# NightShade99/Self-Supervised-Vision

Hardware: AMD Instinct MI355X
Metric: images/sec (whole node) SimCLR ResNet-50 two-view train step (higher is better)
Workload: dtype f32; 1 GPU; SimCLR resnet50 (7x7/2 stem) synthetic 3x224x224, bs=512/GPU, global batch 512, NT-Xent(normalize, T=0.5) over the global batch, SGD-Nesterov; per_gpu_batch=512, global_batch=512, params=27971008, parallelism=single, view_streams=2, library=self-supervised-vision_amd/csrc/libssv_hip.so

## Files before the change

### include/ssv_hip.h

```cpp
#ifndef SSV_HIP_H
#define SSV_HIP_H

#include <stddef.h>
#include <stdint.h>

#ifdef __cplusplus
extern "C" {
#endif

typedef enum ssv_status {
  SSV_OK = 0,
  SSV_ERR_INVALID = -1,
  SSV_ERR_WORKSPACE = -2,
  SSV_ERR_LAUNCH = -3
} ssv_status;

int ssv_version(void);
const char* ssv_last_error(void);
const char* ssv_source_sha16(void);
int ssv_device_cus(void);

typedef struct ssv_conv_desc {
  int32_t N, H, W, C;
  int32_t K, R, S;
  int32_t stride, pad;
  int32_t Ho, Wo;
  int32_t arithmetic;
  int32_t reserved;
  const void* w_planes;
} ssv_conv_desc;
enum { SSV_ARITH_F32_MFMA = 0, SSV_ARITH_BF16X3 = 6 };
int ssv_conv_arithmetic(const ssv_conv_desc* d, int32_t product);
int ssv_split_planes(int64_t n, const float* x, void* planes, void* stream);

int ssv_conv2d_fwd(const ssv_conv_desc* d, const float* x, const float* w, const float* bias,
                   const float* addend, float* y, void* stream);
int ssv_pad_channels(int64_t npix, int32_t cin, int32_t cout, const float* in, float* out, int32_t accumulate, void* stream);
int ssv_group_expand(int32_t K, int32_t R, int32_t S, int32_t Cg, int32_t groups, const float* wg, float* wd, void* stream);
int ssv_group_extract(int32_t K, int32_t R, int32_t S, int32_t Cg, int32_t groups, const float* dwd, float* dwg, int32_t accumulate, void* stream);

int ssv_conv2d_fwd_grouped(const ssv_conv_desc* d, int32_t groups, const float* x, const float* wd, const float* bias, const float* addend,
                           float* y, void* stream);
int ssv_conv2d_dgrad_grouped(const ssv_conv_desc* d, int32_t groups, const float* dy, const float* wd, const float* addend, float* dx, void* stream);
size_t ssv_conv2d_wgrad_grouped_workspace_bytes(const ssv_conv_desc* d, int32_t groups);
int ssv_conv2d_wgrad_grouped(const ssv_conv_desc* d, int32_t groups, const float* x, const float* dy, float* dwd, int accumulate,
                             void* ws, size_t ws_bytes, void* stream);
int ssv_filter_transpose(int32_t K, int32_t R, int32_t S, int32_t C, const float* w, float* wt, void* stream);
int64_t ssv_conv2d_fwd_stats_groups(const ssv_conv_desc* d);
int ssv_conv2d_fwd_stats(const ssv_conv_desc* d, const float* x, const float* w, float* y, float* pmean, float* pm2, void* stream);
int ssv_conv2d_fwd_bnrelu_in_stats(const ssv_conv_desc* d, const float* x, const float* in_scale, const float* in_shift,
                                   const float* w, float* y, float* pmean, float* pm2, void* stream);
int ssv_conv2d_wgrad_bnrelu_in(const ssv_conv_desc* d, const float* x, const float* in_scale, const float* in_shift, const float* dy,
                               float* dw, int accumulate, void* ws, size_t ws_bytes, void* stream);
typedef struct ssv_bn_gate {
  const float* x;
  const float* scale;
  const float* shift;
  const uint8_t* mask;
  const float* mean;
  const float* invstd;
  float* psum_g;
  float* psum_gx;
  const float* x2;
  const float* mean2;
  const float* invstd2;
// ... 274 lines not shown
```

### self-supervised-vision_amd/_lib.py

```python
import ctypes as C
import os

import torch

_HERE = os.path.dirname(os.path.abspath(__file__))
LIB_PATH = os.environ.get("SSV_HIP_LIB") or os.path.join(_HERE, "csrc", "libssv_hip.so")

ABI_VERSION = 121
PROF_CLASSES = ("conv_fwd", "conv_dgrad", "conv_wgrad", "bn_fwd", "bn_bwd", "pool", "loss", "optim", "aug", "misc", "attn", "norm")


class SsvError(RuntimeError):
    pass


ARITH_F32_MFMA, ARITH_BF16X3 = 0, 6


class ConvDesc(C.Structure):
    _fields_ = [(n, C.c_int32) for n in ("N", "H", "W", "C", "K", "R", "S", "stride", "pad", "Ho", "Wo", "arithmetic", "reserved")] + [("w_planes", C.c_void_p)]


class BnGate(C.Structure):
    _fields_ = [(n, C.c_void_p) for n in ("x", "scale", "shift", "mask", "mean", "invstd", "psum_g", "psum_gx", "x2", "mean2", "invstd2", "psum_gx2")]


class BnDyin(C.Structure):
    _fields_ = [(n, C.c_void_p) for n in ("x", "coef")]


class AugCfg(C.Structure):
    _fields_ = [(n, C.c_double) for n in ("brightness", "contrast", "saturation", "hue", "p_jitter", "p_gray", "p_flip",
                                          "scale_min", "scale_max", "ratio_min", "ratio_max")]


_vp, _i32, _i64, _f32, _sz = C.c_void_p, C.c_int32, C.c_int64, C.c_float, C.c_size_t
_u64 = C.c_uint64
_f3 = C.POINTER(C.c_float)
_cd = C.POINTER(ConvDesc)

SIGNATURES = {
    "ssv_version": (C.c_int, []),
    "ssv_last_error": (C.c_char_p, []),
    "ssv_source_sha16": (C.c_char_p, []),
    "ssv_device_cus": (C.c_int, []),
    "ssv_conv2d_fwd": (C.c_int, [_cd, _vp, _vp, _vp, _vp, _vp, _vp]),
    "ssv_pad_channels": (C.c_int, [_i64, _i32, _i32, _vp, _vp, _i32, _vp]),
    "ssv_group_expand": (C.c_int, [_i32, _i32, _i32, _i32, _i32, _vp, _vp, _vp]),
    "ssv_group_extract": (C.c_int, [_i32, _i32, _i32, _i32, _i32, _vp, _vp, _i32, _vp]),
    "ssv_conv2d_fwd_stats_groups": (_i64, [_cd]),
    "ssv_conv2d_fwd_stats": (C.c_int, [_cd, _vp, _vp, _vp, _vp, _vp, _vp]),
    "ssv_conv2d_fwd_bnrelu_in_stats": (C.c_int, [_cd, _vp, _vp, _vp, _vp, _vp, _vp, _vp, _vp]),
    "ssv_conv2d_fwd_sumin_stats": (C.c_int, [_cd] + [_vp] * 13),
    "ssv_conv2d_wgrad_bnrelu_in": (C.c_int, [_cd, _vp, _vp, _vp, _vp, _vp, C.c_int, _vp, _sz, _vp]),
    "ssv_bn_stats_finalize": (C.c_int, [_i64, _i32, _vp, _vp, _i32, _vp, _vp, _f32, _f32, _vp, _vp, _vp, _vp, _vp, _vp, _vp, _vp, _sz, _vp]),
    "ssv_bn_apply": (C.c_int, [_i64, _i32, _vp, _vp, _vp, _vp, _vp, _vp, C.c_int, _vp, _vp, _vp]),
    "ssv_bn_relu_bwd_affine": (C.c_int, [_i64, _i32, _vp, _vp, _vp, _vp, _vp, _vp, _vp, _vp, _vp, _vp, C.c_int, _vp, _sz, _vp]),
    "ssv_bn_train_fwd_partials": (C.c_int, [_i64, _i32, _vp, _vp, _vp, _i32, _vp, _vp, _vp, C.c_int, _f32, _f32, _vp, _vp, _vp, _vp, _vp, _vp, _vp, _vp, _sz, _vp]),
    "ssv_filter_transpose": (C.c_int, [_i32, _i32, _i32, _i32, _vp, _vp, _vp]),
    "ssv_conv2d_dgrad": (C.c_int, [_cd, _vp, _vp, _vp, _vp, _vp]),
    "ssv_conv2d_fwd_gate_groups": (_i64, [_cd]),
    "ssv_conv2d_fwd_gated": (C.c_int, [_cd, _vp, _vp, _vp, _vp, C.POINTER(BnGate), _vp]),
    "ssv_conv2d_fwd_gated_s2add": (C.c_int, [_cd, _vp, _vp, _vp, _i32, _i32, _vp, C.POINTER(BnGate), _vp]),
    "ssv_conv2d_fwd_dyin_s2add": (C.c_int, [_cd, _vp, C.POINTER(BnDyin), _vp, _vp, _i32, _i32, _vp, C.POINTER(BnGate), _vp]),
    "ssv_conv2d_dgrad_gate_groups": (_i64, [_cd]),
    "ssv_conv2d_dgrad_gated": (C.c_int, [_cd, _vp, _vp, _vp, _vp, C.POINTER(BnGate), _vp]),
    "ssv_bn_bwd_from_partials": (C.c_int, [_i64, _i32, _vp, _vp, _vp, _vp, _vp, _vp, _vp, _i64, _vp, _vp, _vp, C.c_int, _vp, _sz, _vp]),
    "ssv_bn_bwd_coef": (C.c_int, [_i64, _i32, _vp, _vp, _vp, _vp, _vp, _i64, _vp, _vp, _vp, C.c_int, _vp, _sz, _vp]),
    "ssv_conv2d_fwd_dyin": (C.c_int, [_cd, _vp, C.POINTER(BnDyin), _vp, _vp, _vp, C.POINTER(BnGate), _vp]),
    "ssv_conv2d_wgrad_dyin": (C.c_int, [_cd, _vp, _vp, _vp, _vp, C.POINTER(BnDyin), _vp, C.c_int, _vp, _sz, _vp]),
    "ssv_conv2d_wgrad_workspace_bytes": (_sz, [_cd]),
    "ssv_conv2d_fwd_grouped": (C.c_int, [_cd, _i32, _vp, _vp, _vp, _vp, _vp, _vp]),
    "ssv_conv2d_dgrad_grouped": (C.c_int, [_cd, _i32, _vp, _vp, _vp, _vp, _vp]),
    "ssv_conv2d_wgrad_grouped_workspace_bytes": (_sz, [_cd, _i32]),
    "ssv_conv2d_wgrad_grouped": (C.c_int, [_cd, _i32, _vp, _vp, _vp, C.c_int, _vp, _sz, _vp]),
    "ssv_conv2d_wgrad": (C.c_int, [_cd, _vp, _vp, _vp, C.c_int, _vp, _sz, _vp]),
    "ssv_conv2d_wgrad_bias_workspace_bytes": (_sz, [_cd]),
    "ssv_conv2d_wgrad_bias": (C.c_int, [_cd, _vp, _vp, _vp, _vp, C.c_int, _vp, _sz, _vp]),
    "ssv_stem_conv_fwd": (C.c_int, [_cd, _vp, _vp, _vp, _vp, _vp, _vp]),
    "ssv_stem_conv_fwd_stats_rows_per_group": (_i64, [_cd]),
    "ssv_stem_conv_wgrad_rows_per_group": (_i64, [_cd]),
    "ssv_stem_conv_wgrad_workspace_bytes": (_sz, [_cd]),
    "ssv_stem_conv_wgrad": (C.c_int, [_cd, _vp, _vp, _vp, _vp, _sz, _vp]),
# ... 204 lines not shown
```

### self-supervised-vision_amd/csrc/conv_mfma.hip

```cpp
#include "common.h"
#include "split_bf16.h"
#include <string.h>
#include <type_traits>

namespace {

constexpr int GBK = 16;

__device__ __forceinline__ int xcd_remap(int orig, int nwg) {
  const int q = nwg >> 3, r = nwg & 7, xcd = orig & 7;
  return (xcd < r ? xcd * (q + 1) : r * (q + 1) + (xcd - r) * q) + (orig >> 3);
}

struct ConvKP {
  int N, H, W, C, K, R, S, stride, pad, Ho, Wo;
  int M;
  int RSC;
  FastDiv dHoWo, dWo, dC, dS, dWp;
  float* aux_out;
  float* aux_out2;
  const float* aux_in;
  const float* xf_scale;
  const float* xf_shift;
  ssv_bn_gate gate;
  const float* dyin_x;
  const float* dyin_coef;
  const float* sum_res; const float* sum_scale; const float* sum_shift; const float* sum_rscale; const float* sum_rshift;
  float* sum_out; uint8_t* sum_mask;
  long long bs_a, bs_b, bs_o;
  int add_H2, add_W2;
  int Cg, Kg;
  const unsigned short* w_planes;
  long long wp_stride;
};

__device__ __forceinline__ void group_span(int n0, int n1, int og, int ig, int bk, int ctot, int& lo, int& hi) {
  const int glo = n0 / og, ghi = (n1 - 1) / og;
  lo = glo * ig / bk * bk;
  hi = min(ctot, ((ghi + 1) * ig + bk - 1) / bk * bk);
}

constexpr int XF_MAXC = 1024;

__device__ __forceinline__ float gelu_f(float v) { return ssv_gelu(v); }
__device__ __forceinline__ float gelu_grad_f(float v) { return ssv_gelu_grad(v); }

using rsrc_t = __amdgpu_buffer_rsrc_t;
constexpr int OOB_OFF = (int)0x80000000u;
__device__ __forceinline__ rsrc_t make_rsrc(const void* base, unsigned bytes) {
  return __builtin_amdgcn_make_buffer_rsrc((void*)base, 0, bytes, 0x00020000);
}
// ... 846 lines not shown
        }
      } else {
        epilogue_vec<TM, TN, EPI>(sel_acc<(SP != 0)>(acc, acc16), smem + wave * (32 * (TN * 32 + 4)), lane, n0 + wc0, p.K, bias, addend, y, (long long)p.M * p.K,
                                  [&](int r) -> long long { const int m = rbase + r; return m < p.M ? (long long)m * p.K : -1; },
                                  (EPI == 1 || EPI == 4) ? p.aux_out : nullptr, (EPI == 2 || EPI == 5) ? p.aux_in : nullptr);
      }
      return;
    }
  }
  static_assert(GATE == 0 || (VEC && EP_FLOATS <= SMEM), "the gated epilogue is the vectorised one");
  if constexpr (SP) return;
  const int l31 = lane & 31, h = lane >> 5;
#pragma unroll
  for (int tn = 0; tn < TN; ++tn) {
    const int col = n0 + wc0 + tn * 32 + l31;
    if (col >= p.K) continue;
    const float bv = bias ? bias[col] : 0.f;
#pragma unroll
    for (int tm = 0; tm < TM; ++tm) {
#pragma unroll
      for (int j = 0; j < 16; ++j) {
        const int row = m0 + wr0 + tm * 32 + (j & 3) + 8 * (j >> 2) + 4 * h;
        if (row < p.M) {
          const size_t o = (size_t)row * p.K + col;
          float v = acc[tm][tn][j] + bv;
          if (addend) v += addend[o];
          y[o] = v;
        }
      }
    }
  }
}

template <int BM, int BN, int WGM, int WGN, int BK, bool EPI = false, int GATE = 0, bool SP = false>
__global__ void __launch_bounds__(256, SP ? 2 : 3)
conv_dgrad_k(ConvKP p, const float* __restrict__ dy, const float* __restrict__ w, const float* addend, float* dx) {
  constexpr int TM = BM / WGM / 32, TN = BN / WGN / 32;
  constexpr int LDT = BK + 4;
  static_assert(!SP || (BK == 32 && BN == 128), "the bf16-piece data gradient: K-step 32, 128 input channels per tile");
  constexpr int A_FLOATS = BM * LDT, B_FLOATS = BK * BN, STAGE = SP ? 48 * (BM + BN) : A_FLOATS + B_FLOATS;
  __shared__ __attribute__((aligned(16))) float smem[STAGE];
  __shared__ unsigned rowpix[BM];
  __shared__ int taps[64 * 3];
  __shared__ int ntaps_s;
  float* As = smem;
  float* Bs = smem + A_FLOATS;
  const int tid = threadIdx.x, lane = tid & 63, wave = tid >> 6;
  const int wr0 = (wave / WGN) * (BM / WGM), wc0 = (wave % WGN) * (BN / WGN);
  const int st = p.stride;
  const int ph = blockIdx.y / st, pw = blockIdx.y - ph * st;
  const int Hq = ph < p.H ? (p.H - ph + st - 1) / st : 0;
  const int Wq = pw < p.W ? (p.W - pw + st - 1) / st : 0;
  const int Mc = p.N * Hq * Wq;
  const int NT = (p.C + BN - 1) / BN;
  const int bid = xcd_remap(blockIdx.x, gridDim.x);
  const int mt = bid / NT, nt = bid - mt * NT;
  const int m0 = mt * BM, n0 = nt * BN;
  if (m0 >= Mc) {
    if constexpr (GATE != 0) {
      const long long grp = ((long long)blockIdx.y * (gridDim.x / NT) + mt) * (BM / 64) + (wr0 / 64);
      const int col = n0 + wc0 + lane;
      for (int c = col; c < min(n0 + wc0 + BN / WGN, p.C); c += 64) { p.gate.psum_g[grp * p.C + c] = 0.f; p.gate.psum_gx[grp * p.C + c] = 0.f; }
    }
    return;
  }

// ... 453 lines not shown
      const float c = partial[(size_t)(k + 2) * n + i], d = partial[(size_t)(k + 3) * n + i];
      s += (a + b) + (c + d);
    }
    for (; k < k1; ++k) s += partial[(size_t)k * n + i];
  }
  sm[grp][e] = s;
  __syncthreads();
  if (grp == 0 && i < n) dw[i] = (accumulate ? dw[i] : 0.f) + ((sm[0][e] + sm[1][e]) + (sm[2][e] + sm[3][e]));
}

int check_desc(const ssv_conv_desc* d, const char* who) {
  SSV_REQUIRE(d != nullptr, "%s: null descriptor", who);
  SSV_REQUIRE(d->N > 0 && d->H > 0 && d->W > 0 && d->C > 0 && d->K > 0 && d->R > 0 && d->S > 0 && d->stride > 0 && d->pad >= 0,
              "%s: non-positive dimension", who);
  const int Ho = (d->H + 2 * d->pad - d->R) / d->stride + 1, Wo = (d->W + 2 * d->pad - d->S) / d->stride + 1;
  SSV_REQUIRE(Ho == d->Ho && Wo == d->Wo, "%s: Ho/Wo (%d,%d) inconsistent with input/filter/stride/pad (expect %d,%d)", who, d->Ho, d->Wo, Ho, Wo);
  SSV_REQUIRE((int64_t)d->N * d->H * d->W < (1ll << 31) && (int64_t)d->N * d->Ho * d->Wo < (1ll << 31), "%s: too many pixels", who);
  SSV_REQUIRE((int64_t)d->R * d->S * d->C < (1 << 24) && d->R * d->S <= 64 && d->H < 32768 && d->W < 32768, "%s: filter too large", who);
  SSV_REQUIRE((int64_t)d->N * d->H * d->W * d->C < (1ll << 29) - (1 << 22) && (int64_t)d->N * d->Ho * d->Wo * d->K < (1ll << 29) - (1 << 22) &&
              (int64_t)d->K * d->R * d->S * d->C < (1ll << 29), "%s: tensor of 2 GiB or more - split the batch", who);
  return SSV_OK;
}

ConvKP make_kp(const ssv_conv_desc* d) {
  ConvKP p;
  p.N = d->N; p.H = d->H; p.W = d->W; p.C = d->C; p.K = d->K; p.R = d->R; p.S = d->S;
  p.stride = d->stride; p.pad = d->pad; p.Ho = d->Ho; p.Wo = d->Wo;
  p.M = d->N * d->Ho * d->Wo;
  p.RSC = d->R * d->S * d->C;
  p.dHoWo = make_fastdiv((uint32_t)(d->Ho * d->Wo));
  p.dWo = make_fastdiv((uint32_t)d->Wo);
  p.dC = make_fastdiv((uint32_t)d->C);
  p.dS = make_fastdiv((uint32_t)d->S);
  p.dWp = make_fastdiv((uint32_t)d->W + 2u);
  p.aux_out = nullptr; p.aux_out2 = nullptr; p.aux_in = nullptr; p.xf_scale = nullptr; p.xf_shift = nullptr;
  memset(&p.gate, 0, sizeof(p.gate));
  p.dyin_x = nullptr; p.dyin_coef = nullptr;
  p.sum_res = p.sum_scale = p.sum_shift = p.sum_rscale = p.sum_rshift = nullptr; p.sum_out = nullptr; p.sum_mask = nullptr;
  p.bs_a = p.bs_b = p.bs_o = 0;
  p.add_H2 = p.add_W2 = 0;
  p.Cg = p.Kg = 0;
  p.w_planes = (const unsigned short*)d->w_planes;
  p.wp_stride = (long long)d->K * p.RSC;
  return p;
}

struct RowSplit { int nsplit, chunk; };
RowSplit wgrad_row_split(int bm, int64_t tiles, int64_t rows, int max_chunk = 0) {
  const int slots = bm == 128 ? 768 : 1024;
  int64_t ns = slots / tiles;
  const int64_t max_by_rows = cdiv64(rows, 256);
  if (ns > max_by_rows) ns = max_by_rows;
  if (ns < 1) ns = 1;
  int64_t chunk = cdiv64(cdiv64(rows, ns), 32) * 32;
  if (max_chunk > 0 && chunk > max_chunk) {
    const int64_t nb = cdiv64(rows, (int64_t)max_chunk);
    chunk = cdiv64(cdiv64(rows, nb), 32) * 32;
  }
  return {(int)cdiv64(rows, chunk), (int)chunk};
}

struct WgradPlan { int bm, bn, it, jt, nsplit, chunk; };
WgradPlan plan_wgrad(const ssv_conv_desc* d, int groups = 0) {
  WgradPlan w;
  const int RSC = d->R * d->S * d->C;
  const int64_t M = (int64_t)d->N * d->Ho * d->Wo;
  const bool bd = groups > 1 && d->C % 64 == 0;
// ... 14 lines not shown

}

namespace {

template <int V> using ic = std::integral_constant<int, V>;
template <int V0, int... Vs, class F>
inline void for_value(int v, F&& f) {
  if constexpr (sizeof...(Vs) == 0) f(ic<V0>{});
  else if (v == V0) f(ic<V0>{});
  else for_value<Vs...>(v, f);
}

inline bool sp_planes_fit(const ssv_conv_desc* d) {
  return (int64_t)d->K * d->R * d->S * d->C * 6 < (1ll << 31);
}
inline bool sp_fwd_ok(const ssv_conv_desc* d) {
  return d->arithmetic == SSV_ARITH_BF16X3 && d->w_planes != nullptr && (((uintptr_t)d->w_planes) & 15) == 0 && d->C % 32 == 0 && d->K % 4 == 0 &&
         sp_planes_fit(d);
}
constexpr int SP_DUAL_FROM = 1152;
inline int sp_fwd_mode(const ssv_conv_desc* d) {
  if (!sp_fwd_ok(d)) return 0;
  return (int64_t)d->R * d->S * d->C > SP_DUAL_FROM ? 2 : 1;
}
inline bool sp_dgrad_ok(const ssv_conv_desc* d) {
  return d->arithmetic == SSV_ARITH_BF16X3 && d->w_planes != nullptr && (((uintptr_t)d->w_planes) & 15) == 0 && d->K % 32 == 0 && d->C >= 128 && d->C % 8 == 0 &&
         sp_planes_fit(d);
}
inline bool sp_wgrad_ok(const ssv_conv_desc* d) {
  return d->arithmetic == SSV_ARITH_BF16X3 && d->C % 4 == 0 && d->K % 4 == 0;
}

struct FwdTile { int bm, bn, sp; unsigned grid_x; };
inline FwdTile fwd_tile(const ssv_conv_desc* d, int groups = 0) {
  FwdTile t;
  t.sp = sp_fwd_mode(d);
  const bool wide = d->K >= 128 && groups <= 1;
  t.bm = (wide || t.sp) ? 128 : 256;
  t.bn = wide ? 128 : 64;
  t.grid_x = (unsigned)(cdiv64((int64_t)d->N * d->Ho * d->Wo, t.bm) * cdiv(d->K, t.bn));
  return t;
}

enum { ARITH_ANY, ARITH_F32, ARITH_SPLIT };

struct FwdArgs { FwdTile t; unsigned batch; hipStream_t s; const ConvKP* p; const float* x; const float* w; const float* bias; const float* addend; float* y; };

template <int BK, int EPI = 0, bool STATS = false, int C4 = 0, bool XF = false, int GATE = 0, int OPM = 0, bool ADDS2 = false,
          int ARITH = (C4 != 0 || BK != 32) ? ARITH_F32 : ARITH_ANY>
inline void fwd_launch(const FwdArgs& a) {
  constexpr bool wide_only = ADDS2 || EPI != 0;
  auto arith = [&](auto SP) {
    auto tile = [&](auto BM, auto BN, auto WGM, auto WGN) {
      hipLaunchKernelGGL((conv_fwd_k<decltype(BM)::value, decltype(BN)::value, decltype(WGM)::value, decltype(WGN)::value, BK, true, EPI, STATS, C4, XF, GATE, OPM, ADDS2, decltype(SP)::value>),
                         dim3(a.t.grid_x, a.batch), dim3(256), 0, a.s, *a.p, a.x, a.w, a.bias, a.addend, a.y);
    };
    if (wide_only || a.t.bn == 128) tile(ic<128>{}, ic<128>{}, ic<2>{}, ic<2>{});
    else if constexpr (wide_only) {}
    else if constexpr (decltype(SP)::value != 0) tile(ic<128>{}, ic<64>{}, ic<2>{}, ic<2>{});
    else tile(ic<256>{}, ic<64>{}, ic<4>{}, ic<1>{});
  };
  if constexpr (ARITH == ARITH_F32) for_value<0>(a.t.sp, arith);
  else if constexpr (ARITH == ARITH_SPLIT) for_value<2, 1>(a.t.sp, arith);
  else for_value<2, 1, 0>(a.t.sp, arith);
}

int launch_fwd(const ssv_conv_desc* d, const float* x, const float* w, const float* bias, const float* addend, float* y,
               float* pmean, float* pm2, const float* in_scale, const float* in_shift, hipStream_t s, const ssv_bn_gate* gate = nullptr,
               int add_H2 = 0, int add_W2 = 0, int groups = 0) {
  ConvKP p = make_kp(d);
  p.add_H2 = add_H2; p.add_W2 = add_W2;
  p.aux_out = pmean; p.aux_out2 = pm2; p.xf_scale = in_scale; p.xf_shift = in_shift;
  if (groups > 1) { p.Cg = d->C / groups; p.Kg = d->K / groups; }
  if (gate) p.gate = *gate;
  const bool stats = pmean != nullptr, xf = in_scale != nullptr;
  const FwdArgs a = {fwd_tile(d, groups), 1, s, &p, x, w, bias, addend, y};
  if (gate) {
    const int gm = gate->x2 ? 3 : (gate->mask ? 2 : 1);
    if (add_H2 > 0) for_value<3, 2>(gm, [&](auto G) { fwd_launch<32, 0, false, 0, false, decltype(G)::value, 0, true>(a); });
    else for_value<3, 2, 1>(gm, [&](auto G) { fwd_launch<32, 0, false, 0, false, decltype(G)::value>(a); });
  }
  else if (stats && d->C == 4) fwd_launch<32, 0, true, 1>(a);
  else if (stats && xf) fwd_launch<32, 0, true, 0, true>(a);
  else if (stats) fwd_launch<32, 0, true>(a);
// ... 120 lines not shown
}

extern "C" int ssv_conv2d_fwd_dyin(const ssv_conv_desc* d, const float* g, const ssv_bn_dyin* dyin, const float* w, const float* addend, float* y,
                                   const ssv_bn_gate* gate, void* stream) {
  return fwd_dyin_impl(d, g, dyin, w, addend, 0, 0, y, gate, stream);
}

extern "C" int ssv_conv2d_fwd_dyin_s2add(const ssv_conv_desc* d, const float* g, const ssv_bn_dyin* dyin, const float* w, const float* addend,
                                         int32_t H2, int32_t W2, float* y, const ssv_bn_gate* gate, void* stream) {
  SSV_REQUIRE(d && gate && gate->mask && addend && d->K >= 128, "ssv_conv2d_fwd_dyin_s2add: needs the compact addend, the byte-mask gate and K >= 128");
  SSV_REQUIRE(H2 == (d->Ho + 1) / 2 && W2 == (d->Wo + 1) / 2, "ssv_conv2d_fwd_dyin_s2add: the compact addend must be ceil(Ho/2) x ceil(Wo/2) (got %d x %d for %d x %d)", H2, W2, d->Ho, d->Wo);
  return fwd_dyin_impl(d, g, dyin, w, addend, H2, W2, y, gate, stream);
}

extern "C" int ssv_conv2d_fwd_sumin_stats(const ssv_conv_desc* d, const float* x, const float* res, const float* scale, const float* shift,
                                          const float* rscale, const float* rshift, const float* w, float* y, float* pmean, float* pm2,
                                          float* a_out, uint8_t* mask_out, void* stream) {
  if (int rc = check_desc(d, "ssv_conv2d_fwd_sumin_stats")) return rc;
  SSV_REQUIRE(x && res && scale && shift && w && y && pmean && pm2 && a_out, "ssv_conv2d_fwd_sumin_stats: null pointer");
  SSV_REQUIRE((rscale == nullptr) == (rshift == nullptr), "ssv_conv2d_fwd_sumin_stats: rscale / rshift must both be given or both NULL");
  SSV_REQUIRE((((uintptr_t)x | (uintptr_t)res | (uintptr_t)scale | (uintptr_t)shift | (uintptr_t)rscale | (uintptr_t)rshift | (uintptr_t)w | (uintptr_t)y |
                (uintptr_t)pmean | (uintptr_t)pm2 | (uintptr_t)a_out) & 15) == 0, "ssv_conv2d_fwd_sumin_stats: pointers must be 16-byte aligned");
  SSV_REQUIRE(d->R == 1 && d->S == 1 && d->stride == 1 && d->pad == 0 && d->C % 32 == 0 && d->K % 4 == 0,
              "ssv_conv2d_fwd_sumin_stats: a 1x1 / stride-1 / unpadded convolution with C %% 32 == 0 and K %% 4 == 0 (got %dx%d s%d p%d C=%d K=%d)",
              d->R, d->S, d->stride, d->pad, d->C, d->K);
  hipStream_t s = (hipStream_t)stream;
  ProfScope ps(SSV_PROF_CONV_FWD, s);
  ConvKP p = make_kp(d);
  p.aux_out = pmean; p.aux_out2 = pm2;
  p.sum_res = res; p.sum_scale = scale; p.sum_shift = shift; p.sum_rscale = rscale; p.sum_rshift = rshift; p.sum_out = a_out; p.sum_mask = mask_out;
  fwd_launch<32, 0, true, 0, false, 0, 2>({fwd_tile(d), 1, s, &p, x, w, nullptr, nullptr, y});
  SSV_CHECK_LAUNCH("ssv_conv2d_fwd_sumin_stats");
  return SSV_OK;
}

extern "C" int64_t ssv_conv2d_fwd_stats_groups(const ssv_conv_desc* d) {
  return d ? cdiv64((int64_t)d->N * d->Ho * d->Wo, 64) : 0;
}

extern "C" int ssv_conv2d_fwd_stats(const ssv_conv_desc* d, const float* x, const float* w, float* y, float* pmean, float* pm2, void* stream) {
  return ssv_conv2d_fwd_bnrelu_in_stats(d, x, nullptr, nullptr, w, y, pmean, pm2, stream);
}

extern "C" int ssv_conv2d_fwd_bnrelu_in_stats(const ssv_conv_desc* d, const float* x, const float* in_scale, const float* in_shift,
                                              const float* w, float* y, float* pmean, float* pm2, void* stream) {
  if (int rc = check_desc(d, "ssv_conv2d_fwd_bnrelu_in_stats")) return rc;
  SSV_REQUIRE(x && w && y, "ssv_conv2d_fwd_bnrelu_in_stats: null pointer");
  SSV_REQUIRE((pmean == nullptr) == (pm2 == nullptr), "ssv_conv2d_fwd_bnrelu_in_stats: pmean / pm2 must both be given or both NULL");
  SSV_REQUIRE((in_scale == nullptr) == (in_shift == nullptr), "ssv_conv2d_fwd_bnrelu_in_stats: in_scale / in_shift must both be given or both NULL");
  SSV_REQUIRE(pmean || in_scale, "ssv_conv2d_fwd_bnrelu_in_stats: neither statistics nor a fused input requested - call ssv_conv2d_fwd");
  SSV_REQUIRE((((uintptr_t)x | (uintptr_t)w | (uintptr_t)y | (uintptr_t)pmean | (uintptr_t)pm2 | (uintptr_t)in_scale | (uintptr_t)in_shift) & 15) == 0,
              "ssv_conv2d_fwd_bnrelu_in_stats: pointers must be 16-byte aligned");
  SSV_REQUIRE((d->C % 32 == 0 || (d->C == 4 && !in_scale)) && d->K % 4 == 0,
              "ssv_conv2d_fwd_bnrelu_in_stats: needs C %% 32 == 0 (or the 4-channel stem, statistics only) and K %% 4 == 0 (got C=%d K=%d)", d->C, d->K);
  SSV_REQUIRE(!in_scale || d->C <= XF_MAXC, "ssv_conv2d_fwd_bnrelu_in_stats: a fused input supports at most %d channels (got %d)", XF_MAXC, d->C);
  hipStream_t s = (hipStream_t)stream;
  ProfScope ps(SSV_PROF_CONV_FWD, s);
  launch_fwd(d, x, w, nullptr, nullptr, y, pmean, pm2, in_scale, in_shift, s);
  SSV_CHECK_LAUNCH("ssv_conv2d_fwd_bnrelu_in_stats");
  return SSV_OK;
}

namespace {
struct DgradTile { int bm, bn, bk; bool sp; int64_t row_tiles; dim3 grid; };
inline DgradTile dgrad_tile(const ssv_conv_desc* d, int groups = 0) {
  DgradTile t;
// ... 706 lines not shown
```

### self-supervised-vision_amd/csrc/runtime.hip

```cpp
#include "common.h"
#include <atomic>
#include <mutex>
#include <vector>
#include <string.h>

static thread_local char g_err[512] = "";

void ssv_set_error(const char* fmt, ...) {
  va_list ap; va_start(ap, fmt);
  vsnprintf(g_err, sizeof(g_err), fmt, ap);
  va_end(ap);
}

extern "C" int ssv_version(void) { return 121; }
extern "C" const char* ssv_last_error(void) { return g_err; }
#ifndef SSV_SRC_SHA16
#define SSV_SRC_SHA16 "unknown"
#endif
extern "C" const char* ssv_source_sha16(void) { return SSV_SRC_SHA16; }

extern "C" int ssv_device_cus(void) {
  int dev = 0;
  if (hipGetDevice(&dev) != hipSuccess) return 0;
  hipDeviceProp_t prop;
  if (hipGetDeviceProperties(&prop, dev) != hipSuccess) return 0;
  return prop.multiProcessorCount;
}

struct ProfRec { int cls; hipEvent_t a, b; bool closed; };
static std::atomic<bool> g_prof_on{false};
static std::mutex g_prof_mu;
static std::vector<ProfRec> g_recs;
static std::vector<ProfRec> g_free;
static uint64_t g_gen = 0;
static thread_local int g_open = -1;
static thread_local uint64_t g_open_gen = 0;

void ssv_prof_begin(int cls, hipStream_t s) {
  if (!g_prof_on.load(std::memory_order_relaxed)) return;
  std::lock_guard<std::mutex> lock(g_prof_mu);
  ProfRec r;
  if (!g_free.empty()) { r = g_free.back(); g_free.pop_back(); }
  else { (void)hipEventCreate(&r.a); (void)hipEventCreate(&r.b); }
  r.cls = cls;
  r.closed = false;
  (void)hipEventRecord(r.a, s);
  g_recs.push_back(r);
// ... 60 lines not shown
```

### self-supervised-vision_amd/csrc/split_bf16.h

```cpp
#pragma once
#include "common.h"

typedef __bf16 bf16x8 __attribute__((ext_vector_type(8)));
typedef __bf16 bf16x2 __attribute__((ext_vector_type(2)));
typedef short s16x4 __attribute__((ext_vector_type(4)));
typedef unsigned u32x4 __attribute__((ext_vector_type(4)));
typedef unsigned u32x2 __attribute__((ext_vector_type(2)));
typedef float f32x2 __attribute__((ext_vector_type(2)));

namespace splitbf {

constexpr int BK = 32;
constexpr int ROWB = 2 * BK;

__device__ __forceinline__ void split4(const f32x4& v, u32x2 (&pl)[3]) {
  f32x2 x0 = {v[0], v[1]}, x1 = {v[2], v[3]};
#pragma unroll
  for (int q = 0; q < 3; ++q) {
    const unsigned p0 = __builtin_bit_cast(unsigned, __builtin_convertvector(x0, bf16x2)), p1 = __builtin_bit_cast(unsigned, __builtin_convertvector(x1, bf16x2));
    if (q < 2) {
      x0 -= f32x2{__uint_as_float(p0 << 16), __uint_as_float(p0 & 0xFFFF0000u)};
      x1 -= f32x2{__uint_as_float(p1 << 16), __uint_as_float(p1 & 0xFFFF0000u)};
    }
    pl[q] = u32x2{p0, p1};
  }
}

__device__ __forceinline__ int rowk_off(int row, int slot) { return row * ROWB + ((slot ^ (((row >> 3) & 1) * 3)) << 4); }

__device__ __forceinline__ void rowk_store(unsigned char* img, int plane_bytes, int row, int k4, const f32x4& v) {
  u32x2 pl[3];
  split4(v, pl);
  const int off = rowk_off(row, k4 >> 1) + (k4 & 1) * 8;
#pragma unroll
  for (int q = 0; q < 3; ++q) *reinterpret_cast<u32x2*>(img + q * plane_bytes + off) = pl[q];
}

__device__ __forceinline__ bf16x8 rowk_frag(const unsigned char* plane, int row0, int lane) {
  return *reinterpret_cast<const bf16x8*>(plane + rowk_off(row0 + (lane & 15), lane >> 4));
}

template <int RB>
__device__ __forceinline__ int krow_off(int m, int chunk) {
  static_assert(RB == 256 || RB == 128, "KROW rows are 128 or 64 channels");
  if constexpr (RB == 256) return m * 256 + ((chunk ^ (((m & 3) << 2) | ((m >> 2) & 3))) << 4);
  else return m * 128 + ((chunk ^ ((((m >> 1) & 1) | (((m >> 3) & 1) << 1)) << 1)) << 4);
}

template <int RB>
__device__ __forceinline__ void krow_store(unsigned char* img, int plane_bytes, int m, int ch, const f32x4& v) {
  u32x2 pl[3];
  split4(v, pl);
  const int off = krow_off<RB>(m, ch >> 3) + ((ch >> 2) & 1) * 8;
#pragma unroll
  for (int q = 0; q < 3; ++q) *reinterpret_cast<u32x2*>(img + q * plane_bytes + off) = pl[q];
}

template <int RB>
__device__ __forceinline__ bf16x8 krow_frag(const unsigned char* plane, int ch0, int lane) {
  const int jl = lane & 15, q = jl >> 2, pp = jl & 3, kg = lane >> 4;
  const int chunk = (ch0 >> 3) + (pp >> 1);
  typedef __attribute__((address_space(3))) s16x4* lds_p;
  const s16x4 lo = __builtin_amdgcn_ds_read_tr16_b64_v4i16((lds_p)(plane + krow_off<RB>(8 * kg + q, chunk) + 8 * (pp & 1)));
  const s16x4 hi = __builtin_amdgcn_ds_read_tr16_b64_v4i16((lds_p)(plane + krow_off<RB>(8 * kg + 4 + q, chunk) + 8 * (pp & 1)));
  typedef short s16x8 __attribute__((ext_vector_type(8)));
  const s16x8 v = {lo[0], lo[1], lo[2], lo[3], hi[0], hi[1], hi[2], hi[3]};
  return __builtin_bit_cast(bf16x8, v);
}

__device__ __forceinline__ void mma6(f32x4& acc, const bf16x8 (&col)[3], const bf16x8 (&row)[3]) {
#define SSV_MM(P, Q) acc = __builtin_amdgcn_mfma_f32_16x16x32_bf16(col[P], row[Q], acc, 0, 0, 0)
  SSV_MM(2, 0); SSV_MM(0, 2); SSV_MM(1, 1); SSV_MM(1, 0); SSV_MM(0, 1); SSV_MM(0, 0);
// ... 11 lines not shown
```

### self-supervised-vision_amd/ops.py

```python
import ctypes as C
import math
import os

import torch

from . import _lib
from ._lib import ConvDesc, call, ptr, stream, workspace

BN_EPS = 1e-5
BN_MOMENTUM = 0.1


def _empty(shape, like):
    return torch.empty(shape, dtype=torch.float32, device=like.device)


ARITHMETIC = os.environ.get("SSV_ARITHMETIC", "bf16x3")
if ARITHMETIC not in ("bf16x3", "f32"):
    raise _lib.SsvError(f"SSV_ARITHMETIC must be bf16x3 or f32 (got {ARITHMETIC!r})")


class arithmetic:

    def __init__(self, name):
        if name not in ("bf16x3", "f32"):
            raise _lib.SsvError(f"arithmetic must be bf16x3 or f32 (got {name!r})")
        self.name = name

    def __enter__(self):
        global ARITHMETIC
        self.prev, ARITHMETIC = ARITHMETIC, self.name
        invalidate_weight_caches()
        return self

    def __exit__(self, *exc):
        global ARITHMETIC
        ARITHMETIC = self.prev
        invalidate_weight_caches()
        return False


def conv_desc(x_shape, w_shape, stride, pad, w=None):
    n, h, w_, c = x_shape
    k, ci, r, s = w_shape
    if ci != c:
        raise _lib.SsvError(f"conv: input has {c} channels, filter expects {ci}")
    ho, wo = (h + 2 * pad - r) // stride + 1, (w_ + 2 * pad - s) // stride + 1
    d = ConvDesc(n, h, w_, c, k, r, s, stride, pad, ho, wo)
    if ARITHMETIC == "bf16x3":
        d.arithmetic = _lib.ARITH_BF16X3
        if w is not None and w.numel() % 8 == 0 and (c % 32 == 0 or k % 32 == 0):
            d.w_planes = ptr(_planes(w))
    return d


def _ohwi(w):
    if w.dim() == 2:
        if not w.is_contiguous():
            raise _lib.SsvError("linear weight must be contiguous")
        return w, (w.shape[0], w.shape[1], 1, 1)
    if not w.is_contiguous(memory_format=torch.channels_last):
        raise _lib.SsvError("conv filter must be in channels_last (OHWI) memory format")
    return w, tuple(w.shape)


_MAX_ELEMS = (1 << 29) - (1 << 22)


def _batch_chunks(n, per_sample_elems, rows_per_sample=None):
    worst = max(per_sample_elems)
    if n * worst < _MAX_ELEMS:
        return [(0, n)]
    nc = (_MAX_ELEMS - 1) // worst
    if nc < 1:
        raise _lib.SsvError("a single sample exceeds the 2 GiB per-launch tensor limit of the convolution kernels")
    if rows_per_sample is not None:
        q = 64 // math.gcd(rows_per_sample, 64)
        if nc // q * q < 1:
            raise _lib.SsvError(f"the statistics epilogue needs chunks of a multiple of {q} samples ({rows_per_sample} output rows per sample) but only "
                                f"{nc} sample(s) fit below the 2 GiB per-launch tensor limit: run this layer without the fused statistics "
                                f"(SSV_NO_BN_STATS_FUSION=1) or with smaller images")
# ... 1301 lines not shown
```

Measured before the change: 2910 images/sec.

## Add staged-row 3x3 stride-1 forward conv kernel reusing input halo across taps

Adds a specialized forward kernel for 3x3/stride1/pad1 convolutions with K<=64 in bf16x3 mode. It stages a contiguous window of input rows (tile plus halo) into LDS once per channel chunk and reuses it for all nine taps, using per-row tap masks and a zero pad region instead of reloading im2col patches per tap. This cuts global loads for the input operand, at the cost of more LDS and a narrow applicability condition. A context manager and a descriptor flag allow falling back to the generic loader.

```diff
diff --git a/include/ssv_hip.h b/include/ssv_hip.h
--- a/include/ssv_hip.h
+++ b/include/ssv_hip.h
@@ -30,7 +30,9 @@
   const void* w_planes;
 } ssv_conv_desc;
 enum { SSV_ARITH_F32_MFMA = 0, SSV_ARITH_BF16X3 = 6 };
+enum { SSV_CONV_GENERIC_LOADER = 1 };
 int ssv_conv_arithmetic(const ssv_conv_desc* d, int32_t product);
+int64_t ssv_conv_fwd_staged_rows(const ssv_conv_desc* d);
 int ssv_split_planes(int64_t n, const float* x, void* planes, void* stream);
 
 int ssv_conv2d_fwd(const ssv_conv_desc* d, const float* x, const float* w, const float* bias,
diff --git a/self-supervised-vision_amd/_lib.py b/self-supervised-vision_amd/_lib.py
--- a/self-supervised-vision_amd/_lib.py
+++ b/self-supervised-vision_amd/_lib.py
@@ -6,7 +6,7 @@
 _HERE = os.path.dirname(os.path.abspath(__file__))
 LIB_PATH = os.environ.get("SSV_HIP_LIB") or os.path.join(_HERE, "csrc", "libssv_hip.so")
 
-ABI_VERSION = 121
+ABI_VERSION = 122
 PROF_CLASSES = ("conv_fwd", "conv_dgrad", "conv_wgrad", "bn_fwd", "bn_bwd", "pool", "loss", "optim", "aug", "misc", "attn", "norm")
 
 
@@ -15,6 +15,7 @@
 
 
 ARITH_F32_MFMA, ARITH_BF16X3 = 0, 6
+CONV_GENERIC_LOADER = 1
 
 
 class ConvDesc(C.Structure):
@@ -49,6 +50,7 @@
     "ssv_group_expand": (C.c_int, [_i32, _i32, _i32, _i32, _i32, _vp, _vp, _vp]),
     "ssv_group_extract": (C.c_int, [_i32, _i32, _i32, _i32, _i32, _vp, _vp, _i32, _vp]),
     "ssv_conv2d_fwd_stats_groups": (_i64, [_cd]),
+    "ssv_conv_fwd_staged_rows": (_i64, [_cd]),
     "ssv_conv2d_fwd_stats": (C.c_int, [_cd, _vp, _vp, _vp, _vp, _vp, _vp]),
     "ssv_conv2d_fwd_bnrelu_in_stats": (C.c_int, [_cd, _vp, _vp, _vp, _vp, _vp, _vp, _vp, _vp]),
     "ssv_conv2d_fwd_sumin_stats": (C.c_int, [_cd] + [_vp] * 13),
diff --git a/self-supervised-vision_amd/csrc/conv_mfma.hip b/self-supervised-vision_amd/csrc/conv_mfma.hip
--- a/self-supervised-vision_amd/csrc/conv_mfma.hip
+++ b/self-supervised-vision_amd/csrc/conv_mfma.hip
@@ -16,7 +16,7 @@
   int N, H, W, C, K, R, S, stride, pad, Ho, Wo;
   int M;
   int RSC;
-  FastDiv dHoWo, dWo, dC, dS, dWp;
+  FastDiv dHoWo, dWo, dC, dS;
   float* aux_out;
   float* aux_out2;
   const float* aux_in;
@@ -929,6 +929,151 @@
   }
 }
 
+constexpr int S3_ROWS = 256;
+constexpr int S3_ZROWS = 8;
+__host__ __device__ inline int s3_rows(int W) { return 130 + 2 * W; }
+
+template <bool STATS, bool XF, int GATE>
+__global__ void __launch_bounds__(256, 2)
+conv_fwd3x3_k(ConvKP p, const float* __restrict__ x, const float* __restrict__ w, const float* __restrict__ bias, const float* addend, float* y) {
+  constexpr int BM = 128, BN = 64, TM = 2, TN = 1;
+  constexpr int A_PLANE = (S3_ROWS + S3_ZROWS) * splitbf::ROWB, B_PLANE = BN * splitbf::ROWB, B_STAGE = 3 * B_PLANE;
+  constexpr int SMEM = (3 * A_PLANE + 2 * B_STAGE) / 4;
+  static_assert(SMEM >= 4 * 32 * (TN * 32 + 4), "the epilogue's slabs reuse the operand images");
+  __shared__ __attribute__((aligned(16))) float smem[SMEM];
+  unsigned char* const Asb = reinterpret_cast<unsigned char*>(smem);
+  unsigned char* const Bsb = Asb + 3 * A_PLANE;
+  const int tid = threadIdx.x, lane = tid & 63, wave = tid >> 6;
+  const int wr0 = (wave >> 1) * 64, wc0 = (wave & 1) * 32;
+  const int m0 = xcd_remap(blockIdx.x, gridDim.x) * BM;
+
+  f32x4 acc16[2 * TM][2 * TN];
+#pragma unroll
+  for (int i = 0; i < 2 * TM; ++i)
+#pragma unroll
+    for (int j = 0; j < 2 * TN; ++j) acc16[i][j] = f32x4{0.f, 0.f, 0.f, 0.f};
+
+  unsigned tapok[2 * TM];
+#pragma unroll
+  for (int i = 0; i < 2 * TM; ++i) {
+    const int m = m0 + wr0 + 16 * i + (lane & 15);
+    unsigned v = 0;
+    if (m < p.M) {
+      const uint32_t n = fdiv((uint32_t)m, p.dHoWo);
+      const uint32_t rem = (uint32_t)m - n * (uint32_t)(p.H * p.W);
+      const uint32_t h = fdiv(rem, p.dWo);
+      const uint32_t wx = rem - h * (uint32_t)p.W;
+      const unsigned sm = (wx > 0 ? 1u : 0u) | 2u | ((int)wx < p.W - 1 ? 4u : 0u);
+      v = (h > 0 ? sm : 0u) | (sm << 3) | ((int)h < p.H - 1 ? sm << 6 : 0u);
+    }
+    tapok[i] = v;
+  }
+
+  const long long wplane = p.wp_stride;
+  const rsrc_t rwp = make_rsrc(p.w_planes, (unsigned)((2 * wplane + (long long)p.K * p.RSC) * 2));
+  const int boffp = (tid >> 2) < p.K ? ((tid >> 2) * p.RSC + (tid & 3) * 8) * 2 : OOB_OFF;
+  const int bldsp = splitbf::rowk_off(tid >> 2, tid & 3);
+  u32x4 rbp[3];
+  auto load_b = [&](int tap, int c0) {
+#pragma unroll
+    for (int q = 0; q < 3; ++q)
+      rbp[q] = (u32x4)__builtin_amdgcn_raw_buffer_load_b128(rwp, boffp == OOB_OFF ? OOB_OFF : boffp + q * (int)(wplane * 2), (tap * p.C + c0) * 2, 0);
+  };
+  auto store_b = [&](int stage) {
+#pragma unroll
+    for (int q = 0; q < 3; ++q) *reinterpret_cast<u32x4*>(Bsb + stage * B_STAGE + q * B_PLANE + bldsp) = rbp[q];
+  };
+
+  constexpr int NPASS = S3_ROWS / 32;
+  const int k4 = tid & 7, rsub = tid >> 3;
+  const int nrows = s3_rows(p.W), npass = (nrows + 31) >> 5;
+  const rsrc_t rx = make_rsrc(x, (unsigned)p.M * p.C * 4u);
+  const rsrc_t rxs0 = make_rsrc(XF ? p.xf_scale : x, XF ? (unsigned)p.C * 4u : 16u), rxs1 = make_rsrc(XF ? p.xf_shift : x, XF ? (unsigned)p.C * 4u : 16u);
+  int aoff[NPASS];
+#pragma unroll
+  for (int i = 0; i < NPASS; ++i) {
+    const int row = rsub + 32 * i, pm = m0 - p.W - 1 + row;
+    aoff[i] = (row < nrows && pm >= 0 && pm < p.M) ? (pm * p.C + 4 * k4) * 4 : OOB_OFF;
+  }
+  f32x4 ra[NPASS], co[XF ? 2 : 1];
+  auto load_a = [&](int c0) {
+    if constexpr (XF) { co[0] = bload4(rxs0, k4 * 16, c0 * 4); co[1] = bload4(rxs1, k4 * 16, c0 * 4); }
+#pragma unroll
+    for (int i = 0; i < NPASS; ++i)
+      if (i < npass) ra[i] = bload4(rx, aoff[i], c0 * 4);
+  };
+  auto store_a = [&]() {
+#pragma unroll
+    for (int i = 0; i < NPASS; ++i) {
+      if (i < npass) {
+        f32x4 v = ra[i];
+        if constexpr (XF) {
+          const float cap = aoff[i] != OOB_OFF ? __builtin_inff() : 0.f;
+#pragma unroll
+          for (int e = 0; e < 4; ++e) v[e] = __builtin_amdgcn_fmed3f(__builtin_fmaf(v[e], co[0][e], co[1][e]), 0.f, cap);
+        }
+        splitbf::rowk_store_any(Asb, A_PLANE, rsub + 32 * i, k4, v);
+      }
+    }
+  };
+  auto mma_tap = [&](int tap, int roff, const unsigned char* Bs) {
+    bf16x8 fb[2 * TN][3];
+#pragma unroll
+    for (int j = 0; j < 2 * TN; ++j)
+#pragma unroll
+      for (int q = 0; q < 3; ++q) fb[j][q] = splitbf::rowk_frag(Bs + q * B_PLANE, wc0 + 16 * j, lane);
+#pragma unroll
+    for (int i = 0; i < 2 * TM; ++i) {
+      const int row = wr0 + 16 * i + (lane & 15) + roff;
+      const int off = splitbf::rowk_off_any(((tapok[i] >> tap) & 1u) ? row : S3_ROWS + (row & (S3_ZROWS - 1)), lane >> 4);
+      bf16x8 fa[3];
+#pragma unroll
+      for (int q = 0; q < 3; ++q) fa[q] = *reinterpret_cast<const bf16x8*>(Asb + q * A_PLANE + off);
+#pragma unroll
+      for (int j = 0; j < 2 * TN; ++j) splitbf::mma6(acc16[i][j], fb[j], fa);
+    }
+  };
+
+  if (tid < 3 * S3_ZROWS * 4) {
+    const int q = tid / (S3_ZROWS * 4), piece = tid % (S3_ZROWS * 4);
+    *reinterpret_cast<u32x4*>(Asb + q * A_PLANE + S3_ROWS * splitbf::ROWB + piece * 16) = u32x4{0u, 0u, 0u, 0u};
+  }
+  const int nchunk = p.C >> 5;
+  load_b(0, 0);
+  load_a(0);
+  store_a();
+  store_b(0);
+  __syncthreads();
+  int stage = 0;
+  for (int c = 0; c < nchunk; ++c) {
+    const bool more = c + 1 < nchunk;
+#pragma unroll
+    for (int tap = 0; tap < 9; ++tap) {
+      load_b(tap == 8 ? 0 : tap + 1, (tap == 8 ? c + 1 : c) * 32);
+      if (tap == 0 && more) load_a((c + 1) * 32);
+      mma_tap(tap, (tap / 3) * p.W + tap % 3, Bsb + stage * B_STAGE);
+      stage ^= 1;
+      store_b(stage);
+      __syncthreads();
+    }
+    if (more) { store_a(); __syncthreads(); }
+  }
+
+  const int rbase = m0 + wr0;
+  float* const ep = smem + wave * (32 * (TN * 32 + 4));
+  auto row_off = [&](int r) -> long long { const int m = rbase + r; return m < p.M ? (long long)m * p.K : -1; };
+  if constexpr (STATS) {
+    const int valid = min(64, p.M - rbase);
+    epilogue_vec<TM, TN, 0, true>(acc16, ep, lane, wc0, p.K, bias, addend, y, (long long)p.M * p.K, row_off,
+                                  nullptr, nullptr, p.aux_out + (size_t)(rbase / 64) * p.K, p.aux_out2 + (size_t)(rbase / 64) * p.K, valid > 0 ? valid : 0);
+  } else if constexpr (GATE != 0) {
+    epilogue_vec<TM, TN, 0, false, GATE>(acc16, ep, lane, wc0, p.K, bias, addend, y, (long long)p.M * p.K, row_off,
+                                         nullptr, nullptr, nullptr, nullptr, 0, &p.gate, (long long)(rbase / 64));
+  } else {
+    epilogue_vec<TM, TN, 0>(acc16, ep, lane, wc0, p.K, bias, addend, y, (long long)p.M * p.K, row_off);
+  }
+}
+
 template <int BM, int BN, int WGM, int WGN, int BK, bool EPI = false, int GATE = 0, bool SP = false>
 __global__ void __launch_bounds__(256, SP ? 2 : 3)
 conv_dgrad_k(ConvKP p, const float* __restrict__ dy, const float* __restrict__ w, const float* addend, float* dx) {
@@ -1448,7 +1593,6 @@
   p.dWo = make_fastdiv((uint32_t)d->Wo);
   p.dC = make_fastdiv((uint32_t)d->C);
   p.dS = make_fastdiv((uint32_t)d->S);
-  p.dWp = make_fastdiv((uint32_t)d->W + 2u);
   p.aux_out = nullptr; p.aux_out2 = nullptr; p.aux_in = nullptr; p.xf_scale = nullptr; p.xf_shift = nullptr;
   memset(&p.gate, 0, sizeof(p.gate));
   p.dyin_x = nullptr; p.dyin_coef = nullptr;
@@ -1529,7 +1673,7 @@
   return d->arithmetic == SSV_ARITH_BF16X3 && d->C % 4 == 0 && d->K % 4 == 0;
 }
 
-struct FwdTile { int bm, bn, sp; unsigned grid_x; };
+struct FwdTile { int bm, bn, sp, staged; unsigned grid_x; };
 inline FwdTile fwd_tile(const ssv_conv_desc* d, int groups = 0) {
   FwdTile t;
   t.sp = sp_fwd_mode(d);
@@ -1537,6 +1681,8 @@
   t.bm = (wide || t.sp) ? 128 : 256;
   t.bn = wide ? 128 : 64;
   t.grid_x = (unsigned)(cdiv64((int64_t)d->N * d->Ho * d->Wo, t.bm) * cdiv(d->K, t.bn));
+  t.staged = (t.sp == 1 && d->R == 3 && d->S == 3 && d->stride == 1 && d->pad == 1 && d->K <= 64 && groups <= 1 && s3_rows(d->W) <= S3_ROWS &&
+              !(d->reserved & SSV_CONV_GENERIC_LOADER)) ? s3_rows(d->W) : 0;
   return t;
 }
 
@@ -1548,6 +1694,12 @@
           int ARITH = (C4 != 0 || BK != 32) ? ARITH_F32 : ARITH_ANY>
 inline void fwd_launch(const FwdArgs& a) {
   constexpr bool wide_only = ADDS2 || EPI != 0;
+  if constexpr (BK == 32 && EPI == 0 && C4 == 0 && OPM == 0 && !ADDS2 && GATE != 3 && !(GATE != 0 && (STATS || XF)) && ARITH != ARITH_F32) {
+    if (a.t.staged != 0 && a.batch == 1) {
+      hipLaunchKernelGGL((conv_fwd3x3_k<STATS, XF, GATE>), dim3(a.t.grid_x), dim3(256), 0, a.s, *a.p, a.x, a.w, a.bias, a.addend, a.y);
+      return;
+    }
+  }
   auto arith = [&](auto SP) {
     auto tile = [&](auto BM, auto BN, auto WGM, auto WGN) {
       hipLaunchKernelGGL((conv_fwd_k<decltype(BM)::value, decltype(BN)::value, decltype(WGM)::value, decltype(WGN)::value, BK, true, EPI, STATS, C4, XF, GATE, OPM, ADDS2, decltype(SP)::value>),
@@ -1734,6 +1886,11 @@
   fwd_launch<32, 0, true, 0, false, 0, 2>({fwd_tile(d), 1, s, &p, x, w, nullptr, nullptr, y});
   SSV_CHECK_LAUNCH("ssv_conv2d_fwd_sumin_stats");
   return SSV_OK;
+}
+
+extern "C" int64_t ssv_conv_fwd_staged_rows(const ssv_conv_desc* d) {
+  if (check_desc(d, "ssv_conv_fwd_staged_rows")) return 0;
+  return fwd_tile(d).staged;
 }
 
 extern "C" int64_t ssv_conv2d_fwd_stats_groups(const ssv_conv_desc* d) {
diff --git a/self-supervised-vision_amd/csrc/runtime.hip b/self-supervised-vision_amd/csrc/runtime.hip
--- a/self-supervised-vision_amd/csrc/runtime.hip
+++ b/self-supervised-vision_amd/csrc/runtime.hip
@@ -12,7 +12,7 @@
   va_end(ap);
 }
 
-extern "C" int ssv_version(void) { return 121; }
+extern "C" int ssv_version(void) { return 122; }
 extern "C" const char* ssv_last_error(void) { return g_err; }
 #ifndef SSV_SRC_SHA16
 #define SSV_SRC_SHA16 "unknown"
diff --git a/self-supervised-vision_amd/csrc/split_bf16.h b/self-supervised-vision_amd/csrc/split_bf16.h
--- a/self-supervised-vision_amd/csrc/split_bf16.h
+++ b/self-supervised-vision_amd/csrc/split_bf16.h
@@ -38,6 +38,16 @@
 
 __device__ __forceinline__ bf16x8 rowk_frag(const unsigned char* plane, int row0, int lane) {
   return *reinterpret_cast<const bf16x8*>(plane + rowk_off(row0 + (lane & 15), lane >> 4));
+}
+
+__device__ __forceinline__ int rowk_off_any(int row, int slot) { return row * ROWB + ((slot ^ (((row >> 2) & 1) << 1)) << 4); }
+
+__device__ __forceinline__ void rowk_store_any(unsigned char* img, int plane_bytes, int row, int k4, const f32x4& v) {
+  u32x2 pl[3];
+  split4(v, pl);
+  const int off = rowk_off_any(row, k4 >> 1) + (k4 & 1) * 8;
+#pragma unroll
+  for (int q = 0; q < 3; ++q) *reinterpret_cast<u32x2*>(img + q * plane_bytes + off) = pl[q];
 }
 
 template <int RB>
diff --git a/self-supervised-vision_amd/ops.py b/self-supervised-vision_amd/ops.py
--- a/self-supervised-vision_amd/ops.py
+++ b/self-supervised-vision_amd/ops.py
@@ -37,6 +37,25 @@
         global ARITHMETIC
         ARITHMETIC = self.prev
         invalidate_weight_caches()
+        return False
+
+
+GENERIC_LOADER = False
+
+
+class generic_loader:
+
+    def __init__(self, on=True):
+        self.on = bool(on)
+
+    def __enter__(self):
+        global GENERIC_LOADER
+        self.prev, GENERIC_LOADER = GENERIC_LOADER, self.on
+        return self
+
+    def __exit__(self, *exc):
+        global GENERIC_LOADER
+        GENERIC_LOADER = self.prev
         return False
 
 
@@ -47,6 +66,8 @@
         raise _lib.SsvError(f"conv: input has {c} channels, filter expects {ci}")
     ho, wo = (h + 2 * pad - r) // stride + 1, (w_ + 2 * pad - s) // stride + 1
     d = ConvDesc(n, h, w_, c, k, r, s, stride, pad, ho, wo)
+    if GENERIC_LOADER:
+        d.reserved = _lib.CONV_GENERIC_LOADER
     if ARITHMETIC == "bf16x3":
         d.arithmetic = _lib.ARITH_BF16X3
         if w is not None and w.numel() % 8 == 0 and (c % 32 == 0 or k % 32 == 0):
```

Result: no change. 2911 images/sec (median of 2 runs) (+0.0%).
